# 123456jack/decision-making-and-path-planning

Hardware: AMD Instinct MI355X
Metric: planning ticks/sec (batched scenes), 512x512 grid (higher is better)
Workload: dtype f64; 1 GPU; BASELINE configs[1]: 1024 scenes/GPU, 512x512 grid, 64 static obstacles; scenes_per_gpu=1024, global_scenes=1024, grid=512, obstacles=64, parallelism=scene-sharded x1, RCCL scatter/gather outside the timed region, algorithmic_bytes_per_tick=276644

## Files before the change

### decision-making-and-path-planning_amd/csrc/kernels_s.hpp

```cpp
#pragma once
#include <type_traits>
#include "dev_geom.hpp"

#ifndef DMPP_PRIO_T2
#define DMPP_PRIO_T2 12
#define DMPP_PRIO_T3 36
#endif
namespace dmpp {

__device__ __forceinline__ uint64_t mix64(uint64_t v)
{
    uint64_t z = v + 0x9e3779b97f4a7c15ull;
    z = (z ^ (z >> 30)) * 0xbf58476d1ce4e5b9ull;
    z = (z ^ (z >> 27)) * 0x94d049bb133111ebull;
    return z ^ (z >> 31);
}

__device__ __forceinline__ int index_near(double q)
{
    return (int)fmin(fmax(q, -0x1p30), 0x1p30);
}
__device__ __forceinline__ int index_near_hi(double q)
{
    return (int)fmax(fmin(q, 0x1p30), -0x1p30);
}

__device__ __forceinline__ int cell_of(const PlannerConfig& c, GlobalPoint2D origin, double x, double y)
{
    const int ix = clampi(index_near(floor((x - origin.x) / c.cell)), 0, c.grid_w - 1);
    const int iy = clampi(index_near(floor((y - origin.y) / c.cell)), 0, c.grid_h - 1);
    return iy * c.grid_w + ix;
}

__device__ __forceinline__ int hfun(int x, int y, int gx, int gy)
{
    int dx = abs(x - gx), dy = abs(y - gy);
    return 10 * max(dx, dy) + 4 * min(dx, dy);
}

constexpr int kOpenCap = DMPP_OPEN_CAP;
constexpr uint32_t kEntryForcedA = 1u, kEntryForcedB = 2u, kEntryAheadBlocked = 4u;
template <int K> constexpr int closed_log_of() { return K == 2 ? 10 : 9; }
constexpr int kDiagK = DMPP_DIAG_JUMP;
constexpr int kDiagGroup = 2 * kDiagK;
constexpr int kDiagPerRound = DMPP_WAVE / kDiagGroup;
constexpr int kMaxDiag = 16;
constexpr int kSearchSetupWaves = 4, kSearchBlock = kSearchSetupWaves * DMPP_WAVE;
constexpr int kSearchSetupWavesWide = 16;
constexpr int kOrderShift = 13;
constexpr int kOrderClasses = 1024;

constexpr int kGroupMax = 4;
struct TickGroup {
    int n;
    const SceneIn* in;
    const ObPoint* obs_now; long long obs_stride;
    int32_t* paths; long long path_stride;
    GridOut* gout; long long gout_stride;
};

__device__ __forceinline__ uint32_t wave_min_u32(uint32_t v)
{
#define DMPP_DPP_MIN(ctrl, rowmask)                                                                              \
    { const uint32_t t = (uint32_t)__builtin_amdgcn_update_dpp((int)0xFFFFFFFF, (int)v, ctrl, rowmask, 0xf, false); \
      v = t < v ? t : v; }
    DMPP_DPP_MIN(0x111, 0xf) DMPP_DPP_MIN(0x112, 0xf) DMPP_DPP_MIN(0x114, 0xf) DMPP_DPP_MIN(0x118, 0xf)
    DMPP_DPP_MIN(0x142, 0xa) DMPP_DPP_MIN(0x143, 0xc)
#undef DMPP_DPP_MIN
    return (uint32_t)__builtin_amdgcn_readlane((int)v, 63);
}

__device__ __forceinline__ int popc_m(uint32_t v) { return __popc(v); }
__device__ __forceinline__ int popc_m(uint64_t v) { return __popcll(v); }
__device__ __forceinline__ int lsb_m(uint32_t v) { return __ffs((int)v) - 1; }
__device__ __forceinline__ int lsb_m(uint64_t v) { return __ffsll((long long)v) - 1; }
__device__ __forceinline__ int msb_m(uint32_t v) { return 31 - __clz((int)v); }
__device__ __forceinline__ int msb_m(uint64_t v) { return 63 - __clzll((long long)v); }

constexpr uint32_t kLineOutside = 0xFFFFFFFFu;
template <class M> struct LineM { M mask; uint32_t off; };

#define DMPP_LDS __attribute__((address_space(3)))
template <int K>
struct SparseView {
    using M = std::conditional_t<K == 2, uint64_t, uint32_t>;
    DMPP_LDS uint32_t* data; DMPP_LDS unsigned char* meta; DMPP_LDS uint16_t* off2; int LW, NL;

    __device__ __forceinline__ LineM<M> line(int l) const
    {
        LineM<M> r;
        const bool in = (unsigned)l < (unsigned)NL;
        const int li = in ? l : 0;
        if constexpr (K == 0) { const uint32_t v = ((DMPP_LDS const uint32_t*)meta)[li]; r.mask = v & 0xFFFFu; r.off = v >> 16; }
        else if constexpr (K == 1) { r.mask = ((DMPP_LDS const uint32_t*)meta)[2 * li]; r.off = ((DMPP_LDS const uint32_t*)meta)[2 * li + 1]; }
        else { r.mask = ((DMPP_LDS const uint64_t*)meta)[li]; r.off = off2[li]; }
        if (!in) { r.mask = 0; r.off = kLineOutside; }
        return r;
    }
    __device__ __forceinline__ uint32_t word(const LineM<M>& m, int w) const
    {
        const bool outside = m.off == kLineOutside || (unsigned)w >= (unsigned)LW;
        const M bit = (M)1 << (w & (int)(8 * sizeof(M) - 1));
        const bool present = !outside && (m.mask & bit) != 0;
        const uint32_t idx = present ? m.off + (uint32_t)popc_m((M)(m.mask & (bit - 1))) : 0u;
        const uint32_t v = data[idx];
        return outside ? 0xFFFFFFFFu : (present ? v : 0u);
    }
    __device__ __forceinline__ void clear_line(int l) const
    {
        if constexpr (K == 0) ((DMPP_LDS uint32_t*)meta)[l] = 0;
        else if constexpr (K == 1) { ((DMPP_LDS uint32_t*)meta)[2 * l] = 0; ((DMPP_LDS uint32_t*)meta)[2 * l + 1] = 0; }
        else { ((DMPP_LDS uint64_t*)meta)[l] = 0; off2[l] = (uint16_t)0; }
    }
    __device__ __forceinline__ void or_mask(int l, M bits) const
    {
        if constexpr (K == 0) __hip_atomic_fetch_or(&((DMPP_LDS uint32_t*)meta)[l], (uint32_t)bits, __ATOMIC_RELAXED, __HIP_MEMORY_SCOPE_WORKGROUP);
        else if constexpr (K == 1) __hip_atomic_fetch_or(&((DMPP_LDS uint32_t*)meta)[2 * l], (uint32_t)bits, __ATOMIC_RELAXED, __HIP_MEMORY_SCOPE_WORKGROUP);
        else __hip_atomic_fetch_or(&((DMPP_LDS uint64_t*)meta)[l], (uint64_t)bits, __ATOMIC_RELAXED, __HIP_MEMORY_SCOPE_WORKGROUP);
    }
    __device__ __forceinline__ M mask_of(int l) const
    {
        if constexpr (K == 0) return ((DMPP_LDS const uint32_t*)meta)[l] & 0xFFFFu;
        else if constexpr (K == 1) return ((DMPP_LDS const uint32_t*)meta)[2 * l];
        else return ((DMPP_LDS const uint64_t*)meta)[l];
    }
    __device__ __forceinline__ void set_off(int l, uint32_t off) const
    {
        if constexpr (K == 0) ((DMPP_LDS uint32_t*)meta)[l] |= off << 16;
        else if constexpr (K == 1) ((DMPP_LDS uint32_t*)meta)[2 * l + 1] = off;
        else off2[l] = (uint16_t)off;
    }
};
template <int K> __host__ __device__ constexpr int sparse_meta_bytes_per_line() { return K == 0 ? 4 : (K == 1 ? 8 : 10); }

struct DenseView {
    using M = uint64_t;
    const uint32_t* base; DMPP_LDS const uint64_t* nz; int LW, NL;
    __device__ __forceinline__ LineM<M> line(int l) const
    {
        LineM<M> r; r.mask = 0; r.off = kLineOutside;
        if ((unsigned)l < (unsigned)NL) { r.mask = nz[l]; r.off = (uint32_t)(l * LW); }
        return r;
    }
    __device__ __forceinline__ uint32_t word(const LineM<M>& m, int w) const
    {
        if (m.off == kLineOutside || (unsigned)w >= (unsigned)LW) return 0xFFFFFFFFu;
        if (!((m.mask >> w) & 1ull)) return 0u;
        return base[m.off + w];
    }
};

template <class V>
// ... 573 lines not shown
            ospill[base + r] = make_uint2(L.o_ent[slot], f2 | ((uint32_t)L.o_run[slot] << 16));
            L.o_f2[slot] = 0xFFFFu;
            mn = min(mn, f2);
        }
        base += __popcll(bm);
    }
    sp_n = base;
    sp_min = min(sp_min, wave_min_u32(mn));
    __threadfence();
    wave_order();
    return squeeze_open(L, n_open, lane);
}

template <class LDS>
__device__ __forceinline__ int merge_open(LDS& L, int n_open, int lane, uint2* __restrict__ ospill, int& sp_n, uint32_t& sp_min)
{
    n_open = squeeze_open(L, n_open, lane);
    if (kOpenCap - n_open < 2 * DMPP_WAVE) n_open = spill_open(L, n_open, lane, ospill, sp_n, sp_min);
    __threadfence();
    const uint32_t X = sp_min;
    int cntX = 0;
    for (int q0 = 0; q0 < sp_n; q0 += DMPP_WAVE) {
        const int i = q0 + lane;
        const uint32_t f = i < sp_n ? (ospill[i].y & 0xFFFFu) : 0x10000u;
        cntX += __popcll(wave_ballot(f == X));
    }
    const int room = kOpenCap - n_open - DMPP_WAVE;
    const int take = min(cntX, room), skip = cntX - take;
    {
        uint32_t f2[kOpenCap / DMPP_WAVE], ee[kOpenCap / DMPP_WAVE]; uint16_t rr[kOpenCap / DMPP_WAVE];
#pragma unroll
        for (int k = 0; k < kOpenCap / DMPP_WAVE; k++) {
            const int slot = lane + DMPP_WAVE * k;
            f2[k] = 0xFFFFu; ee[k] = 0; rr[k] = 0;
            if (slot < n_open) { f2[k] = L.o_f2[slot]; ee[k] = L.o_ent[slot]; rr[k] = L.o_run[slot]; }
        }
        wave_order();
#pragma unroll
        for (int k = 0; k < kOpenCap / DMPP_WAVE; k++) {
            const int slot = lane + DMPP_WAVE * k;
            if (slot < n_open) { L.o_f2[slot + take] = (uint16_t)f2[k]; L.o_ent[slot + take] = ee[k]; L.o_run[slot + take] = rr[k]; }
        }
        wave_order();
    }
    int r = 0, w = 0; uint32_t nmin = 0xFFFFu;
    for (int q0 = 0; q0 < sp_n; q0 += DMPP_WAVE) {
        const int i = q0 + lane;
        const bool valid = i < sp_n;
        uint2 e = make_uint2(0u, 0xFFFFu);
        if (valid) e = ospill[i];
        const uint32_t f = e.y & 0xFFFFu;
        const bool isX = valid && f == X;
        const unsigned long long bx = wave_ballot(isX);
        const int myr = r + (int)__builtin_amdgcn_mbcnt_hi((unsigned)(bx >> 32), __builtin_amdgcn_mbcnt_lo((unsigned)bx, 0u));
        const bool tk = isX && myr >= skip;
        if (tk) { const int dst = myr - skip; L.o_f2[dst] = (uint16_t)f; L.o_ent[dst] = e.x; L.o_run[dst] = (uint16_t)(e.y >> 16); }
        const bool kp = valid && !tk;
        const unsigned long long bk = wave_ballot(kp);
        if (kp) {
            ospill[w + (int)__builtin_amdgcn_mbcnt_hi((unsigned)(bk >> 32), __builtin_amdgcn_mbcnt_lo((unsigned)bk, 0u))] = e;
            nmin = min(nmin, f);
        }
        r += __popcll(bx); w += __popcll(bk);
    }
    sp_n = w;
    sp_min = wave_min_u32(nmin);
    __threadfence();
    wave_order();
    return n_open + take;
}

template <bool SPILL, class V, class LDS>
__device__ __forceinline__ SearchOut search_core(const PlannerConfig& c, LDS& L, const V& Vrow, const V& Vcol, int start, int goal, int order_cap,
                                        uint32_t* __restrict__ closed, uint16_t* __restrict__ pin, int32_t* __restrict__ order,
                                        int32_t* __restrict__ path, uint2* __restrict__ ospill, int lane
#ifdef DMPP_DEBUG_SEARCH
                                        , long long* dbg_t, int* dbg_c
#endif
                                        )
{
#ifdef DMPP_DEBUG_SEARCH
#define DBG_MARK(slot) { const long long t__ = clock64(); dbg_t[slot] += t__ - dbg_last; dbg_last = t__; }
    long long dbg_last = clock64();
#else
#define DBG_MARK(slot)
#endif
    constexpr int kClosedLog = LDS::kClosedLog, kClosedTab = LDS::kClosedTab, kClosedMax = LDS::kClosedMax;
    using CW = typename LDS::CW;
    const int W = c.grid_w, H = c.grid_h, N = W * H;
    const int gx = goal % W, gy = goal / W;
    const int cap = SPILL ? c.bucket_cap : min(c.bucket_cap, kOpenCap);
    int sp_n = 0; uint32_t sp_min = 0xFFFFu;
    SearchOut R; R.status = -1; R.n_exp = 0; R.n_push = 1; R.n_rounds = 0; R.path_cost = 0; R.path_len = 0; R.digest = 0;
    int status = -1, n_exp = 0, n_rounds = 0, path_cost = 0;
    int my_pushes = 0;
    uint64_t digest = 0;
    bool hash_complete = true;
    int n_open = 1, live = 1, fmax = -1;
    const int s = lane & 7;
    const int sdx = (s == 0 || s == 1 || s == 7) ? 1 : ((s >= 3 && s <= 5) ? -1 : 0);
    const int sdy = (s >= 1 && s <= 3) ? 1 : ((s >= 5) ? -1 : 0);
    const int node = (lane >> 3) & 3;
    const bool is_dscan = lane < 56, bhv = lane >= 28;
    const int bq = bhv ? lane - 28 : lane;
    const int bj = is_dscan ? bq / 7 : 0, bk = is_dscan ? bq % 7 + 1 : 0;
    const int aj = node, ak = (lane & 7) + 1;
    int guard = 16 * N + 1024;
    int steps = 0;
    while (status < 0) {
        if (__builtin_expect(--guard < 0, 0)) { status = DMPP_G_INTERNAL; break; }
        if (steps == DMPP_PRIO_T2) __builtin_amdgcn_s_setprio(2);
        if (steps == DMPP_PRIO_T3) __builtin_amdgcn_s_setprio(3);
        steps++;
#ifdef DMPP_DEBUG_SEARCH
        dbg_c[0]++;
#endif
        if (__builtin_expect((SPILL ? live + sp_n : live) == 0, 0)) { status = DMPP_G_NO_PATH; break; }
        if (__builtin_expect(n_open - live > 64 && n_open > 2 * live, 0)) n_open = squeeze_open(L, n_open, lane);
        const uint32_t v0 = L.o_f2[lane], v1 = L.o_f2[lane + 64], v2 = L.o_f2[lane + 128], v3 = L.o_f2[lane + 192];
        uint32_t v4 = 0xFFFFu, v5 = 0xFFFFu, v6 = 0xFFFFu, v7 = 0xFFFFu;
        const bool upper = n_open > 256;
        if (__builtin_expect(upper, 0)) { v4 = L.o_f2[lane + 256]; v5 = L.o_f2[lane + 320]; v6 = L.o_f2[lane + 384]; v7 = L.o_f2[lane + 448]; }
        const uint32_t fmin2 = wave_min_u32(min(min(min(v0, v1), min(v2, v3)), min(min(v4, v5), min(v6, v7))));
        if constexpr (SPILL) if (__builtin_expect(sp_n > 0 && fmin2 > sp_min, 0)) { n_open = merge_open(L, n_open, lane, ospill, sp_n, sp_min); live = n_open; continue; }
        if (__builtin_expect(fmin2 == 0xFFFFu, 0)) { status = DMPP_G_INTERNAL; break; }
        const int f = (int)fmin2 << 1;
        int nt = 0; unsigned long long sel = 0;
#define DMPP_TAKE(vreg, base)                                                                        \
        {                                                                                            \
            unsigned long long tm = wave_ballot((vreg) == fmin2);                                    \
            while (tm && nt < DMPP_JPS_BATCH) {                                                      \
                const int b = 63 - __clzll((long long)tm);                                           \
                tm &= ~(1ull << b);                                                                  \
                sel |= (unsigned long long)((base) + b) << (16 * nt);                                \
                nt++;                                                                                \
            }                                                                                        \
        }
        if (__builtin_expect(upper, 0)) { DMPP_TAKE(v7, 448) DMPP_TAKE(v6, 384) DMPP_TAKE(v5, 320) DMPP_TAKE(v4, 256) }
        DMPP_TAKE(v3, 192) DMPP_TAKE(v2, 128) DMPP_TAKE(v1, 64) DMPP_TAKE(v0, 0)
#undef DMPP_TAKE
        static_assert(DMPP_JPS_BATCH == 4 && kOpenCap <= 65536, "four 16-bit slot numbers in one 64-bit scalar");
        if constexpr (SPILL) if (__builtin_expect(sp_n > 0 && fmin2 == sp_min && nt < DMPP_JPS_BATCH, 0)) { n_open = merge_open(L, n_open, lane, ospill, sp_n, sp_min); live = n_open; continue; }
        const int i0 = (int)(sel & 0xFFFFu);
        const int myi = (int)((sel >> (16 * node)) & 0xFFFFu);
        const bool have = lane < 32 && node < nt;
        const uint32_t e = L.o_ent[myi]; const int run_in = L.o_run[myi];
        wave_order();
        if (have && s == 0) L.o_f2[myi] = 0xFFFFu;
        live -= nt;
        n_open -= (i0 == n_open - 1) ? 1 : 0;
        const int x = (int)(e & 0xFFFu), y = (int)((e >> 12) & 0xFFFu), d = (int)((e >> 24) & 15u);
        const uint32_t eflags = e >> 28;
        const int cell = y * W + x;
        DBG_MARK(0)
#ifdef DMPP_DEBUG_SEARCH
        dbg_c[1] += nt;
#endif
        const int gcur = f - hfun(x, y, gx, gy);
        bool jump0, diag0;
        {
            const uint32_t row = d >= 8 ? rules::kCodeStart : (uint32_t)((d < 4 ? rules::kCodeLo : rules::kCodeHi) >> ((d & 3) * 16));
            const uint32_t code = (row >> (2 * s)) & 3u;
            jump0 = code == 1u;
            const int rel = (s - d) & 7;
            const bool forced = ((rel <= 2 ? eflags >> 0 : eflags >> 1) & 1u) != 0;
            const bool ahead_free = (eflags & kEntryAheadBlocked) == 0;
            diag0 = (code == 2u && ahead_free) || (code == 3u && forced);
        }
        DBG_MARK(11)
        bool valid = have && s == 0;
        {
            const int c0_ = __builtin_amdgcn_readlane(cell, 0), c1_ = __builtin_amdgcn_readlane(cell, 8), c2_ = __builtin_amdgcn_readlane(cell, 16);
            const bool dup = ((node >= 1) & (cell == c0_)) | ((node >= 2) & (cell == c1_)) | ((node >= 3) & (cell == c2_));
            valid = valid & !dup;
        }
        uint32_t my_slot = 0;
        if (__builtin_expect(n_exp + DMPP_JPS_BATCH <= kClosedMax, 1)) {
            const uint32_t keyc = (uint32_t)cell + 1u;
            uint32_t hh = ((uint32_t)cell * 2654435761u) >> (32 - kClosedLog);
            uint32_t old = 0u;
            if (valid) old = atomicCAS(&L.c_tab[hh], 0u, keyc);
            if (CW::key(old) == keyc) valid = false;
            bool collide = valid && old != 0u;
            for (int probe = 1; probe < kClosedTab && wave_ballot(collide); probe++) {
                if (collide) {
                    hh = (hh + 1) & (kClosedTab - 1);
                    old = atomicCAS(&L.c_tab[hh], 0u, keyc);
                    if (CW::key(old) == keyc) valid = false;
                    collide = old != 0u && CW::key(old) != keyc;
                }
            }
            my_slot = hh;
        } else {
            if (hash_complete) {
                hash_complete = false;
                digest += hash_digest(L, lane);
                uint4* c4 = reinterpret_cast<uint4*>(closed);
                const uint4 z = { 0u, 0u, 0u, 0u };
                for (int i = lane; i < (N >> 7); i += DMPP_WAVE) c4[i] = z;
                __threadfence();
                wave_sync();
                for (int i = lane; i < kClosedTab; i += DMPP_WAVE) {
                    const uint32_t e2 = L.c_tab[i];
                    if (e2) { const int cc = (int)CW::key(e2) - 1; atomicOr(&closed[cc >> 5], 1u << (cc & 31)); pin[cc] = L.c_info[i]; }
                }
                __threadfence();
                wave_sync();
            }
            if (valid) {
                const uint32_t old = atomicOr(&closed[cell >> 5], 1u << (cell & 31));
                if ((old >> (cell & 31)) & 1u) valid = false;
            }
        }
        const bool inserted = valid;
        auto nodes_of = [](unsigned long long bm) { return (((unsigned)bm & 0x01010101u) * 0x01020408u) >> 24; };
        unsigned vm = nodes_of(wave_ballot(valid));
        {
            const int nvb = __popc(vm & ((1u << node) - 1u));
            const unsigned stop = nodes_of(wave_ballot(valid && (cell == goal || n_exp + nvb + 1 >= c.max_expansions)));
            if (__builtin_expect(stop != 0, 0)) {
                const int last = __ffs((int)stop) - 1;
                if (node > last) valid = false;
                vm = nodes_of(wave_ballot(valid));
            }
        }
        {
            const int seq = n_exp + __popc(vm & ((1u << node) - 1u));
            if (inserted && __builtin_expect(hash_complete, 1)) L.c_info[my_slot] = (uint16_t)(d | (run_in << 4));
            if (valid) {
                if (__builtin_expect(!hash_complete, 0)) { pin[cell] = (uint16_t)(d | (run_in << 4)); digest += mix64(((uint64_t)(uint32_t)seq << 32) | (uint32_t)cell); }
                if (order && seq < order_cap) order[seq] = cell;
            }
            if (inserted && __builtin_expect(hash_complete, 1)) L.set_seq(my_slot, valid ? (uint32_t)seq : CW::kSeqNone);
        }
        if (vm && f > fmax) { fmax = f; n_rounds++; }
        n_exp += __popc(vm);
        if (__builtin_expect(wave_ballot(valid && cell == goal) != 0, 0)) { status = DMPP_G_FOUND; path_cost = f; break; }
        if (__builtin_expect(n_exp >= c.max_expansions, 0)) { status = DMPP_G_LIMIT; break; }
        if (__builtin_expect(vm == 0, 0)) continue;
        DBG_MARK(1)
        const bool nvalid = lane < 32 && ((vm >> node) & 1u);
        const bool want_jump = nvalid && jump0, want_diag = nvalid && diag0;
        int run = 0;
        uint32_t nflags = 0;
        DBG_MARK(2)
        const unsigned smask = (unsigned)wave_ballot(want_jump), dmask = (unsigned)wave_ballot(want_diag);
        const int n_sj = __popc(smask), n_dc = __popc(dmask);
        const int my_sj = __popc(smask & ((1u << (lane & 31)) - 1u)), my_dc = __popc(dmask & ((1u << (lane & 31)) - 1u));
        if (want_jump || want_diag) L.job[want_diag ? my_dc : kMaxDiag + my_sj] = (uint32_t)x | ((uint32_t)y << 12) | ((uint32_t)s << 24);
        wave_order();
        const int n_rounds_j = (n_sj | n_dc) ? max(1, (n_dc + 3) >> 2) : 0;
        DBG_MARK(7)
        for (int rnd = 0; rnd < n_rounds_j; rnd++) {
            const int dca = rnd * 4 + aj;
            const bool a_act = lane < 32 && dca < n_dc;
            const uint32_t Ja = L.job[a_act ? dca : 0];
            const int dcb = rnd * 4 + bj;
            const bool b_act = is_dscan ? dcb < n_dc : (rnd == 0 && lane - 56 < n_sj);
            const uint32_t Jb = L.job[b_act ? (is_dscan ? dcb : kMaxDiag + lane - 56) : 0];
            int jl, jp, jsg; bool hv;
            {
                const int ox = (int)(Jb & 0xFFFu), oy = (int)((Jb >> 12) & 0xFFFu), os = (int)(Jb >> 24);
                if (is_dscan) {
                    const int odx = (os == 1 || os == 7) ? 1 : -1, ody = (os == 1 || os == 3) ? 1 : -1;
                    const int cx = ox + bk * odx, cy = oy + bk * ody;
                    hv = bhv; jl = hv ? cx : cy; jp = hv ? cy : cx; jsg = hv ? ody : odx;
                } else {
                    hv = !(os == 0 || os == 4); jsg = (os == 0 || os == 2) ? 1 : -1; jl = hv ? ox : oy; jp = hv ? oy : ox;
                }
            }
            const V vw = hv ? Vcol : Vrow;
            const int aox = (int)(Ja & 0xFFFu), aoy = (int)((Ja >> 12) & 0xFFFu), aos = (int)(Ja >> 24);
            const int aodx = (aos == 1 || aos == 7) ? 1 : -1, aody = (aos == 1 || aos == 3) ? 1 : -1;
            const int acx = aox + ak * aodx, acy = aoy + ak * aody;
            const auto m0 = vw.line(b_act ? jl : -1), mP = vw.line(b_act ? jl + 1 : -1), mM = vw.line(b_act ? jl - 1 : -1);
            const auto r0 = Vrow.line(a_act ? acy : -1), ra = Vrow.line(a_act ? acy + aody : -1), rb = Vrow.line(a_act ? acy - aody : -1);
            DBG_MARK(8)
            bool cblk = false, cstop = false, cf1 = false, cf2 = false;
            {
                const bool b0 = cell_blocked_m(Vrow, r0, acx), b1 = cell_blocked_m(Vrow, r0, acx - aodx), b2 = cell_blocked_m(Vrow, ra, acx - aodx);
                const bool b3 = cell_blocked_m(Vrow, rb, acx), b4 = cell_blocked_m(Vrow, rb, acx + aodx);
                cf1 = a_act & b1 & !b2;
                cf2 = a_act & b3 & !b4;
                cstop = a_act & (b0 | ((acx == gx) & (acy == gy)) | cf1 | cf2);
                cblk = b0 & a_act;
            }
            DBG_MARK(9)
#ifdef DMPP_DEBUG_SEARCH
            const int r = jump_lane(vw, m0, mP, mM, b_act, jl, jp, jsg, hv ? gx : gy, hv ? gy : gx, &dbg_c[2]);
#else
            const int r = jump_lane(vw, m0, mP, mM, b_act, jl, jp, jsg, hv ? gx : gy, hv ? gy : gx);
#endif
            DBG_MARK(10)
            const unsigned long long am = wave_ballot(cstop), kb = wave_ballot(cblk), sb = wave_ballot(is_dscan && r > 0);
            const unsigned long long f1b = wave_ballot(cf1), f2b = wave_ballot(cf2);
            if (want_diag && (my_dc >> 2) == rnd) {
                const int j = my_dc & 3;
                const unsigned ta = (unsigned)(am >> (8 * j)) & 0xFFu, tk = (unsigned)(kb >> (8 * j)) & 0xFFu;
                const unsigned sc = ((unsigned)(sb >> (7 * j)) | (unsigned)(sb >> (28 + 7 * j))) & 0x7Fu;
                const unsigned any = ta | sc;
                const int k1 = any ? __ffs((int)any) - 1 : kDiagK - 1;
                run = ((tk >> k1) & 1u) ? 0 : k1 + 1;
                const unsigned t1 = ((unsigned)(f1b >> (8 * j)) >> k1) & 1u, t2 = ((unsigned)(f2b >> (8 * j)) >> k1) & 1u;
                const unsigned ahead_blk = (tk >> (k1 + 1)) & 1u;
                const bool ccw_is_1 = s == 1 || s == 5;
                nflags = (ccw_is_1 ? t1 : t2) * kEntryForcedA | (ccw_is_1 ? t2 : t1) * kEntryForcedB | ahead_blk * kEntryAheadBlocked;
            }
            const int from_s = __shfl(r, 56 + (my_sj & 7), 64);
            if (rnd == 0 && want_jump) {
                run = from_s & 0xFFF;
                const unsigned fP = ((unsigned)from_s >> 12) & 1u, fM = ((unsigned)from_s >> 13) & 1u;
                const bool ccw_is_p = s == 0 || s == 6;
                nflags = (ccw_is_p ? fP : fM) * kEntryForcedA | (ccw_is_p ? fM : fP) * kEntryForcedB;
            }
        }
        DBG_MARK(3)
#ifdef DMPP_DEBUG_SEARCH
        dbg_c[3] += n_dc; dbg_c[4] += n_rounds_j;
#endif
        const bool push = run > 0;
        const unsigned pm = (unsigned)wave_ballot(push);
        const int cnt = __popc(pm);
        if (__builtin_expect(cnt != 0, 1)) {
            const int nx = x + run * sdx, ny = y + run * sdy;
            const int fn = gcur + run * ((s & 1) ? 14 : 10) + hfun(nx, ny, gx, gy);
            const unsigned rm = (unsigned)wave_ballot(push && fn >= DMPP_F_LIMIT);
            const int live_all = SPILL ? live + sp_n : live;
            if (__builtin_expect(rm || live_all + cnt > cap, 0)) {
                const int k_range = rm ? __popc(pm & ((1u << (__ffs((int)rm) - 1)) - 1u)) : 0x7FFFFFFF;
                const int k_cap = live_all + cnt > cap ? cap - live_all : 0x7FFFFFFF;
                status = k_range <= k_cap ? DMPP_G_COST_RANGE : DMPP_G_OVERFLOW;
                break;
            }
            if (__builtin_expect(n_open + cnt > kOpenCap, 0)) {
                n_open = squeeze_open(L, n_open, lane);
                if constexpr (SPILL) { if (n_open + cnt > kOpenCap) n_open = spill_open(L, n_open, lane, ospill, sp_n, sp_min); live = n_open; }
            }
            if (push) {
                const int slot = n_open + __popc(pm & ((1u << lane) - 1u));
                L.o_f2[slot] = (uint16_t)(fn >> 1);
                L.o_ent[slot] = (uint32_t)nx | ((uint32_t)ny << 12) | ((uint32_t)s << 24) | (nflags << 28);
                L.o_run[slot] = (uint16_t)run;
            }
            n_open += cnt; live += cnt; my_pushes += push ? 1 : 0;
            wave_order();
        }
        DBG_MARK(4)
    }
    DBG_MARK(5)

    if (hash_complete) digest += hash_digest(L, lane);
#pragma unroll
    for (int sft = 32; sft >= 1; sft >>= 1) {
        uint32_t lo = (uint32_t)digest, hi = (uint32_t)(digest >> 32);
        lo = __shfl_xor((int)lo, sft, 64); hi = __shfl_xor((int)hi, sft, 64);
        digest += ((uint64_t)hi << 32) | lo;
    }
    int path_len = 0;
    bool slow_walk = !hash_complete;
    if (status == DMPP_G_FOUND && hash_complete) {
        int Lc = 1, hops = 0, bad = 0;
        if (lane == 0) {
            int cur = goal;
            while (cur != start) {
                if (hops >= kOpenCap) { bad = 2; break; }
                uint32_t hh = ((uint32_t)cur * 2654435761u) >> (32 - kClosedLog);
                int v = -1;
                for (int probe = 0; probe < kClosedTab; probe++) {
                    const uint32_t e2 = L.c_tab[hh]; const int inf = L.c_info[hh];
                    if (CW::key(e2) == (uint32_t)cur + 1u) { v = inf; break; }
                    if (e2 == 0u) break;
                    hh = (hh + 1) & (kClosedTab - 1);
                }
                const int pd = v & 15, rn = v >> 4;
                if (v < 0 || rn == 0 || pd > 7) { bad = 1; break; }
                const int dx = (int)((0x901Au >> (2 * pd)) & 3u) - 1, dy = (int)((0x01A9u >> (2 * pd)) & 3u) - 1;
                const int step = dy * W + dx;
                L.o_ent[hops] = (uint32_t)cur; L.o_run[hops] = (uint16_t)rn; L.o_f2[hops] = (uint16_t)pd;
                hops++; Lc += rn; cur -= rn * step;
            }
        }
        Lc = __builtin_amdgcn_readfirstlane(Lc);
        hops = __builtin_amdgcn_readfirstlane(hops);
        bad = __builtin_amdgcn_readfirstlane(bad);
        wave_sync();
        if (bad == 1) status = DMPP_G_INTERNAL;
        else if (bad == 2) {
            uint4* c4 = reinterpret_cast<uint4*>(closed);
            (void)c4;
            for (int i = lane; i < kClosedTab; i += DMPP_WAVE) {
                const uint32_t e2 = L.c_tab[i];
                if (e2) pin[(int)CW::key(e2) - 1] = L.c_info[i];
            }
            __threadfence();
            wave_sync();
            slow_walk = true;
        } else {
            int keep = Lc;
            if (Lc > c.max_path) { keep = c.max_path; status = DMPP_G_PATH_TRUNC; }
            path_len = keep;
            int kbase = 0;
            for (int j0 = 0; j0 < hops; j0 += DMPP_WAVE) {
                const int j = j0 + lane;
                const int rn = j < hops ? (int)L.o_run[j] : 0;
                int incl = rn;
#pragma unroll
                for (int sft = 1; sft < DMPP_WAVE; sft <<= 1) { const int t = __shfl_up(incl, sft, 64); if (lane >= sft) incl += t; }
                int ec = 0, step = 0;
                const int idx0 = kbase + incl - rn;
                if (rn) {
                    const int pd = L.o_f2[j];
                    ec = (int)L.o_ent[j];
                    const int dx = (int)((0x901Au >> (2 * pd)) & 3u) - 1, dy = (int)((0x01A9u >> (2 * pd)) & 3u) - 1;
                    step = dy * W + dx;
                }
                constexpr int kLongRun = 12;
                if (rn && rn <= kLongRun) { int idx = idx0; for (int r = 0; r < rn && idx < keep; r++, idx++) path[keep - 1 - idx] = ec - r * step; }
                unsigned long long lm = wave_ballot(rn > kLongRun);
                while (lm) {
                    const int src = __ffsll((long long)lm) - 1;
                    lm &= lm - 1;
                    const int h_ec = __shfl(ec, src, 64), h_step = __shfl(step, src, 64), h_rn = __shfl(rn, src, 64), h_idx = __shfl(idx0, src, 64);
                    for (int r = lane; r < h_rn; r += DMPP_WAVE) if (h_idx + r < keep) path[keep - 1 - (h_idx + r)] = h_ec - r * h_step;
                }
                kbase += __shfl(incl, DMPP_WAVE - 1, 64);
            }
            if (lane == 0 && keep == Lc) path[0] = start;
        }
    }
    if (status == DMPP_G_FOUND && slow_walk) {
        int cur = goal, k = 0;
        bool done = false, broken = false;
        while (!done && !broken) {
            int hops = 0;
            if (lane == 0) {
                int kk = k;
                while (cur != start && hops < kOpenCap) {
                    const int v = pin[cur];
                    const int pd = v & 15, rn = v >> 4;
                    if (rn == 0 || pd > 7 || kk > N) { broken = true; break; }
                    const int dx = (pd == 0 || pd == 1 || pd == 7) ? 1 : ((pd >= 3 && pd <= 5) ? -1 : 0);
                    const int dy = (pd >= 1 && pd <= 3) ? 1 : ((pd >= 5) ? -1 : 0);
                    L.o_ent[hops] = (uint32_t)cur; L.o_run[hops] = (uint16_t)rn; L.o_f2[hops] = (uint16_t)pd;
                    hops++; kk += rn;
                    cur -= rn * (dy * W + dx);
                }
                done = cur == start;
            }
            hops = __builtin_amdgcn_readfirstlane(hops);
            cur = __builtin_amdgcn_readfirstlane(cur);
            done = __builtin_amdgcn_readfirstlane((int)done) != 0;
            broken = __builtin_amdgcn_readfirstlane((int)broken) != 0;
            wave_sync();
            for (int j = 0; j < hops; j++) {
                const int ec = (int)L.o_ent[j], rn = L.o_run[j], pd = L.o_f2[j];
                const int dx = (pd == 0 || pd == 1 || pd == 7) ? 1 : ((pd >= 3 && pd <= 5) ? -1 : 0);
                const int dy = (pd >= 1 && pd <= 3) ? 1 : ((pd >= 5) ? -1 : 0);
                const int step = dy * W + dx;
                for (int r = lane; r < rn; r += DMPP_WAVE)
                    if (k + r < c.max_path) path[k + r] = ec - r * step;
                k += rn;
            }
            wave_sync();
        }
        if (broken) { status = DMPP_G_INTERNAL; }
        else {
            if (lane == 0 && k < c.max_path) path[k] = start;
            const int Lc = k + 1;
            int keep = Lc;
            if (Lc > c.max_path) { keep = c.max_path; status = DMPP_G_PATH_TRUNC; }
            path_len = keep;
            wave_sync();
            for (int i = lane; i < keep / 2; i += DMPP_WAVE) {
                const int a0 = path[i], b0 = path[keep - 1 - i];
                path[i] = b0; path[keep - 1 - i] = a0;
            }
        }
    }
    DBG_MARK(6)
    int n_push = my_pushes;
#pragma unroll
    for (int sft = 32; sft >= 1; sft >>= 1) n_push += __shfl_xor(n_push, sft, 64);
    n_push += 1;
    R.status = status; R.n_exp = n_exp; R.n_push = n_push; R.n_rounds = n_rounds; R.path_cost = path_cost; R.path_len = path_len; R.digest = digest;
    return R;
#undef DBG_MARK
}

template <class LDS>
__device__ __forceinline__ void reset_search_lds(LDS& L, int start, int goal, int W, int lane)
{
    for (int i = lane; i < LDS::kClosedTab; i += DMPP_WAVE) L.c_tab[i] = 0;
    for (int i = lane; i < kOpenCap; i += DMPP_WAVE) L.o_f2[i] = 0xFFFFu;
    wave_order();
    if (lane == 0) {
        const int sx = start % W, sy = start / W;
        L.o_ent[0] = (uint32_t)sx | ((uint32_t)sy << 12) | (8u << 24);
        L.o_f2[0] = (uint16_t)(hfun(sx, sy, goal % W, goal / W) >> 1);
        L.o_run[0] = 0;
    }
    wave_order();
}

__device__ __forceinline__ void publish_search(GridOut& go, const SearchOut& R, int start, int goal)
{
    go.order_digest = R.digest; go.status = R.status; go.n_expanded = R.n_exp; go.n_pushed = R.n_push; go.n_rounds = R.n_rounds;
    go.path_len = R.path_len; go.path_cost = R.path_cost; go.start_cell = start; go.goal_cell = goal;
}

#ifdef DMPP_DEBUG_SEARCH
__device__ __forceinline__ void publish_debug(int32_t* path, int max_path, const long long* t, const int* cn, long long t_setup, long long t_total)
{
    int32_t* dbg = path + max_path - 16;
    dbg[0] = cn[0]; dbg[1] = cn[1]; dbg[2] = cn[2]; dbg[3] = cn[3]; dbg[4] = cn[4];
    dbg[5] = (int)(t[0] >> 4); dbg[6] = (int)(t[1] >> 4); dbg[7] = (int)(t[2] >> 4); dbg[8] = (int)(t[3] >> 4); dbg[9] = (int)(t[4] >> 4);
    dbg[10] = (int)(t[6] >> 4); dbg[11] = (int)((t[0] + t[1] + t[2] + t[3] + t[4] + t[5] + t[6]) >> 4); dbg[12] = (int)(t_setup >> 4); dbg[13] = (int)(t_total >> 4);
    dbg[14] = (int)__builtin_amdgcn_s_getreg((31 << 11) | 4);
    dbg[15] = (int)__builtin_amdgcn_s_getreg((31 << 11) | 20);
    for (int i = 7; i < 16; i++) path[max_path - 64 + i] = (int)(t[i] >> 4);
}
#endif

template <int K, int SW, bool SPILL>
__device__ __forceinline__ void search_scene(const PlannerConfig& c, int scene, int w_base, int order_cap, int budget, const SceneIn* __restrict__ in,
         const ObPoint* __restrict__ obs_now, uint32_t* __restrict__ gclosed, uint16_t* __restrict__ pinfo, int32_t* __restrict__ orders,
         int32_t* __restrict__ paths, GridOut* __restrict__ gout, uint32_t* __restrict__ gbitmaps, int32_t* __restrict__ cost_out,
         int32_t* __restrict__ overflow, int32_t* __restrict__ need_max, uint2* __restrict__ ospill_all, int spill_cap,
         int32_t* __restrict__ retry_list, int32_t* __restrict__ retry_cnt,
         SearchLds<closed_log_of<K>()>& L, unsigned char* smem_raw)
{
    using LdsT = SearchLds<closed_log_of<K>()>;
    constexpr unsigned kViewsAt = 0;
    const long long t_begin = clock64();
    const int tid = threadIdx.x, lane = tid & (DMPP_WAVE - 1), wv = tid >> 6;
    const int W = c.grid_w, H = c.grid_h, N = W * H, WW = W >> 5, HW = H >> 5;
    const SceneIn& si = in[scene];
    SparseView<K> vr, vc;
    {
        DMPP_LDS unsigned char* p = (DMPP_LDS unsigned char*)smem_raw + kViewsAt;
        unsigned used = 0;
        if constexpr (K == 2) {
            vr.meta = p; vc.meta = p + (unsigned)H * 8u;
            vr.off2 = (DMPP_LDS uint16_t*)(p + (unsigned)(H + W) * 8u); vc.off2 = vr.off2 + H;
            used = (unsigned)(H + W) * 10u;
        } else {
            constexpr unsigned mb = (unsigned)sparse_meta_bytes_per_line<K>();
            vr.meta = p; vc.meta = p + (unsigned)H * mb;
            vr.off2 = nullptr; vc.off2 = nullptr;
            used = (unsigned)(H + W) * mb;
        }
        used = (used + 15u) & ~15u;
        vr.data = (DMPP_LDS uint32_t*)(p + used); vc.data = vr.data + budget;
        vr.LW = WW; vr.NL = H; vc.LW = HW; vc.NL = W;
    }
    static_assert(sizeof(RasterStage) <= offsetof(LdsT, job), "the staged footprints must fit the open list and the closed set");
    DMPP_LDS RasterStage* stage = (DMPP_LDS RasterStage*)(DMPP_LDS unsigned char*)(unsigned char*)&L;
    int* s_wave2 = (int*)L.job;
    static_assert(sizeof(L.job) >= kSearchSetupWavesWide * sizeof(int), "second row of wave sums");
    const ObPoint* obs = obs_now + si.obs_off;
#ifdef DMPP_DEBUG_SEARCH
    long long tmark[8] = { 0, 0, 0, 0, 0, 0, 0, 0 };
    const int need = budget > 0 ? build_sparse_views<K, SW>(c, si, obs, si.obs_n, vr, vc, budget, stage, L.s_wave, s_wave2, tmark) : 1;
#else
    const int need = budget > 0 ? build_sparse_views<K, SW>(c, si, obs, si.obs_n, vr, vc, budget, stage, L.s_wave, s_wave2) : 1;
#endif
    const bool dense = need > budget;
    if (tid == 0) { if (budget > 0) atomicMax(need_max, need); overflow[scene] = dense ? 1 : 0; }
    uint32_t* bm = gbitmaps + (size_t)scene * 2 * (N >> 5);
    DMPP_LDS uint64_t* nz_row = (DMPP_LDS uint64_t*)((DMPP_LDS unsigned char*)smem_raw + kViewsAt);
    DMPP_LDS uint64_t* nz_col = nz_row + H;
    if (dense) { __syncthreads(); build_dense_views<SW>(c, si, obs, si.obs_n, bm, nz_row, nz_col, stage, L.s_wave); }
    for (int i = tid; i < LdsT::kClosedTab; i += (SW * DMPP_WAVE)) L.c_tab[i] = 0;
    for (int i = tid; i < kOpenCap; i += (SW * DMPP_WAVE)) L.o_f2[i] = 0xFFFFu;
    const DenseView dr{ bm, nz_row, WW, H }, dc{ bm + (N >> 5), nz_col, HW, W };
    const int start = cell_of(c, si.grid_origin, si.loc.globalpoint.x, si.loc.globalpoint.y);
    const int goal = cell_of(c, si.grid_origin, si.goal.x, si.goal.y);
    const bool goal_blocked = dense ? cell_blocked(dr, goal % W, goal / W) : cell_blocked(vr, goal % W, goal / W);
    __syncthreads();
    if (!goal_blocked && tid == 0) {
        const int sx = start % W, sy = start / W;
        if (dense) {
            bm[start >> 5] &= ~(1u << (start & 31));
            bm[(N >> 5) + sx * HW + (sy >> 5)] &= ~(1u << (sy & 31));
            __threadfence();
        } else {
            sparse_clear_cell(vr, sy, sx);
            sparse_clear_cell(vc, sx, sy);
        }
        L.o_ent[0] = (uint32_t)sx | ((uint32_t)sy << 12) | (8u << 24);
        L.o_f2[0] = (uint16_t)(hfun(sx, sy, goal % W, goal / W) >> 1);
        L.o_run[0] = 0;
    }
    __syncthreads();
    int32_t* path = paths + (size_t)scene * c.max_path;
    if (wv != 0) return;
    __builtin_amdgcn_s_setprio(1);
    const long long t_setup = clock64() - t_begin;
    SearchOut R; R.status = DMPP_G_GOAL_BLOCKED; R.n_exp = 0; R.n_push = 0; R.n_rounds = 0; R.path_cost = 0; R.path_len = 0; R.digest = 0;
    uint32_t* closed = gclosed + (size_t)scene * (N >> 5);
    uint16_t* pin = pinfo + (size_t)scene * N;
    int32_t* order = orders ? orders + (size_t)scene * order_cap : nullptr;
    uint2* ospill = ospill_all ? ospill_all + (size_t)scene * spill_cap : nullptr;
// ... 128 lines not shown
```

Measured before the change: 6.382 million ticks/s.

## Parallelize path reconstruction via wave-wide parent-slot table and DPP reductions

Replaces the serial lane-0 hash-probing walk from goal to start with a wave-parallel pass. That pass compacts the occupied closed-hash slots and resolves each slot's parent slot into LDS reused from the open-list arrays, and it also computes the digest in the same sweep. The lane-0 walk then only follows precomputed parent indices, and run lengths and cell coordinates are re-read from the hash table. Shuffle-based reductions and scans are replaced with DPP-based wave scans and sums. The cost is that every search now resolves parents for all occupied slots, not just the ones on the path, and the open-list LDS is aliased for the new tables.

New measurement: 6.487 million ticks/s, median of 6. 1.02x the previous value.

```diff
diff --git a/decision-making-and-path-planning_amd/csrc/kernels_s.hpp b/decision-making-and-path-planning_amd/csrc/kernels_s.hpp
--- a/decision-making-and-path-planning_amd/csrc/kernels_s.hpp
+++ b/decision-making-and-path-planning_amd/csrc/kernels_s.hpp
@@ -68,6 +68,28 @@
     DMPP_DPP_MIN(0x142, 0xa) DMPP_DPP_MIN(0x143, 0xc)
 #undef DMPP_DPP_MIN
     return (uint32_t)__builtin_amdgcn_readlane((int)v, 63);
+}
+
+__device__ __forceinline__ int wave_scan_i32(int v)
+{
+#define DMPP_DPP_ADD(ctrl, rowmask) v += __builtin_amdgcn_update_dpp(0, v, ctrl, rowmask, 0xf, false);
+    DMPP_DPP_ADD(0x111, 0xf) DMPP_DPP_ADD(0x112, 0xf) DMPP_DPP_ADD(0x114, 0xf) DMPP_DPP_ADD(0x118, 0xf)
+    DMPP_DPP_ADD(0x142, 0xa) DMPP_DPP_ADD(0x143, 0xc)
+#undef DMPP_DPP_ADD
+    return v;
+}
+__device__ __forceinline__ int wave_sum_i32(int v) { return __builtin_amdgcn_readlane(wave_scan_i32(v), 63); }
+__device__ __forceinline__ uint64_t wave_sum_u64(uint64_t v)
+{
+#define DMPP_DPP_ADD64(ctrl, rowmask)                                                                             \
+    { const uint32_t lo = (uint32_t)__builtin_amdgcn_update_dpp(0, (int)(uint32_t)v, ctrl, rowmask, 0xf, false);      \
+      const uint32_t hi = (uint32_t)__builtin_amdgcn_update_dpp(0, (int)(uint32_t)(v >> 32), ctrl, rowmask, 0xf, false); \
+      v += ((uint64_t)hi << 32) | lo; }
+    DMPP_DPP_ADD64(0x111, 0xf) DMPP_DPP_ADD64(0x112, 0xf) DMPP_DPP_ADD64(0x114, 0xf) DMPP_DPP_ADD64(0x118, 0xf)
+    DMPP_DPP_ADD64(0x142, 0xa) DMPP_DPP_ADD64(0x143, 0xc)
+#undef DMPP_DPP_ADD64
+    const uint32_t lo = (uint32_t)__builtin_amdgcn_readlane((int)(uint32_t)v, 63), hi = (uint32_t)__builtin_amdgcn_readlane((int)(uint32_t)(v >> 32), 63);
+    return ((uint64_t)hi << 32) | lo;
 }
 
 __device__ __forceinline__ int popc_m(uint32_t v) { return __popc(v); }
@@ -807,6 +829,7 @@
 #ifdef DMPP_DEBUG_SEARCH
 #define DBG_MARK(slot) { const long long t__ = clock64(); dbg_t[slot] += t__ - dbg_last; dbg_last = t__; }
     long long dbg_last = clock64();
+    int hops_dbg = 0;
 #else
 #define DBG_MARK(slot)
 #endif
@@ -821,6 +844,7 @@
     int my_pushes = 0;
     uint64_t digest = 0;
     bool hash_complete = true;
+    uint32_t goal_slot = 0;
     int n_open = 1, live = 1, fmax = -1;
     const int s = lane & 7;
     const int sdx = (s == 0 || s == 1 || s == 7) ? 1 : ((s >= 3 && s <= 5) ? -1 : 0);
@@ -960,7 +984,14 @@
         }
         if (vm && f > fmax) { fmax = f; n_rounds++; }
         n_exp += __popc(vm);
-        if (__builtin_expect(wave_ballot(valid && cell == goal) != 0, 0)) { status = DMPP_G_FOUND; path_cost = f; break; }
+        {
+            const unsigned long long at_goal = wave_ballot(valid && cell == goal);
+            if (__builtin_expect(at_goal != 0, 0)) {
+                status = DMPP_G_FOUND; path_cost = f;
+                goal_slot = (uint32_t)__builtin_amdgcn_readlane((int)my_slot, __ffsll((long long)at_goal) - 1);
+                break;
+            }
+        }
         if (__builtin_expect(n_exp >= c.max_expansions, 0)) { status = DMPP_G_LIMIT; break; }
         if (__builtin_expect(vm == 0, 0)) continue;
         DBG_MARK(1)
@@ -1074,41 +1105,84 @@
     }
     DBG_MARK(5)
 
-    if (hash_complete) digest += hash_digest(L, lane);
-#pragma unroll
-    for (int sft = 32; sft >= 1; sft >>= 1) {
-        uint32_t lo = (uint32_t)digest, hi = (uint32_t)(digest >> 32);
-        lo = __shfl_xor((int)lo, sft, 64); hi = __shfl_xor((int)hi, sft, 64);
-        digest += ((uint64_t)hi << 32) | lo;
-    }
     int path_len = 0;
     bool slow_walk = !hash_complete;
-    if (status == DMPP_G_FOUND && hash_complete) {
+    constexpr uint32_t kParStart = 0xFFFDu, kParInvalid = 0xFFFEu, kParMissing = 0xFFFFu;
+    typedef uint16_t __attribute__((may_alias)) u16_alias;
+    u16_alias* const par = reinterpret_cast<u16_alias*>(L.o_ent);
+    u16_alias* const occ = reinterpret_cast<u16_alias*>(L.o_f2);
+    static_assert(kClosedTab < (int)kParStart && sizeof(L.o_ent) >= kClosedTab * sizeof(uint16_t) && sizeof(L.o_f2) >= kOpenCap * sizeof(uint16_t) &&
+                  offsetof(LDS, o_run) == offsetof(LDS, o_f2) + sizeof(L.o_f2) && sizeof(L.o_f2) + sizeof(L.o_run) >= kClosedTab * sizeof(uint16_t),
+                  "parent slots over o_ent, occupied slots over o_f2 | o_run, the hop list over o_f2");
+    const bool chain = status == DMPP_G_FOUND && hash_complete;
+    const uint32_t start_slot = ((uint32_t)start * 2654435761u) >> (32 - kClosedLog);
+    if (hash_complete) {
+        int n_occ = 0;
+        {
+            constexpr int NS = kClosedTab / DMPP_WAVE;
+            uint32_t E[NS];
+#pragma unroll
+            for (int k = 0; k < NS; k++) E[k] = L.c_tab[lane + k * DMPP_WAVE];
+            wave_order();
+#pragma unroll
+            for (int k = 0; k < NS; k++) {
+                const bool o = E[k] != 0u;
+                const unsigned long long bm = wave_ballot(o);
+                if (o) occ[n_occ + (int)__builtin_amdgcn_mbcnt_hi((unsigned)(bm >> 32), __builtin_amdgcn_mbcnt_lo((unsigned)bm, 0u))] = (uint16_t)(lane + k * DMPP_WAVE);
+                n_occ += __popcll(bm);
+            }
+            wave_order();
+        }
+        for (int r0 = 0; r0 < n_occ; r0 += DMPP_WAVE) {
+            const bool act = r0 + lane < n_occ;
+            const uint32_t sl = act ? (uint32_t)occ[r0 + lane] : 0u;
+            const uint32_t e = L.c_tab[sl], inf = L.c_info[sl]; const uint32_t sq = L.seq_of(sl, e);
+            if (act && sq != CW::kSeqNone) digest += mix64(((uint64_t)sq << 32) | (uint64_t)(CW::key(e) - 1u));
+            if (chain) {
+                const int pd = (int)(inf & 15u), rn = (int)(inf >> 4);
+                const int dx = (int)((0x901Au >> (2 * (pd & 7))) & 3u) - 1, dy = (int)((0x01A9u >> (2 * (pd & 7))) & 3u) - 1;
+                const bool want = act && pd <= 7 && rn > 0;
+                const uint32_t keyc = CW::key(e) - (uint32_t)(rn * (dy * W + dx));
+                uint32_t hh = ((keyc - 1u) * 2654435761u) >> (32 - kClosedLog);
+                uint32_t e2 = L.c_tab[hh];
+                bool miss = want && CW::key(e2) != keyc && e2 == 0u, coll = want && CW::key(e2) != keyc && e2 != 0u;
+                for (int probe = 1; probe < kClosedTab && wave_ballot(coll); probe++) {
+                    if (coll) {
+                        hh = (hh + 1u) & (uint32_t)(kClosedTab - 1);
+                        e2 = L.c_tab[hh];
+                        if (CW::key(e2) == keyc) coll = false;
+                        else if (e2 == 0u) { coll = false; miss = true; }
+                    }
+                }
+                miss |= coll;
+                if (act) par[sl] = (uint16_t)(!want ? kParInvalid : (miss ? kParMissing : (hh == start_slot ? kParStart : hh)));
+            }
+        }
+        wave_order();
+    }
+    DBG_MARK(12)
+    digest = wave_sum_u64(digest);
+    DBG_MARK(15)
+    if (chain) {
         int Lc = 1, hops = 0, bad = 0;
-        if (lane == 0) {
-            int cur = goal;
-            while (cur != start) {
+        if (lane == 0 && goal_slot != start_slot) {
+            uint32_t cur = goal_slot;
+            for (;;) {
+                L.o_f2[hops] = (uint16_t)cur;
+                hops++;
+                const uint32_t up = (uint32_t)__builtin_amdgcn_readfirstlane((int)par[cur]);
+                if (up >= kParStart) { bad = up == kParStart ? 0 : 1; break; }
                 if (hops >= kOpenCap) { bad = 2; break; }
-                uint32_t hh = ((uint32_t)cur * 2654435761u) >> (32 - kClosedLog);
-                int v = -1;
-                for (int probe = 0; probe < kClosedTab; probe++) {
-                    const uint32_t e2 = L.c_tab[hh]; const int inf = L.c_info[hh];
-                    if (CW::key(e2) == (uint32_t)cur + 1u) { v = inf; break; }
-                    if (e2 == 0u) break;
-                    hh = (hh + 1) & (kClosedTab - 1);
-                }
-                const int pd = v & 15, rn = v >> 4;
-                if (v < 0 || rn == 0 || pd > 7) { bad = 1; break; }
-                const int dx = (int)((0x901Au >> (2 * pd)) & 3u) - 1, dy = (int)((0x01A9u >> (2 * pd)) & 3u) - 1;
-                const int step = dy * W + dx;
-                L.o_ent[hops] = (uint32_t)cur; L.o_run[hops] = (uint16_t)rn; L.o_f2[hops] = (uint16_t)pd;
-                hops++; Lc += rn; cur -= rn * step;
-            }
-        }
-        Lc = __builtin_amdgcn_readfirstlane(Lc);
+                cur = up;
+            }
+        }
         hops = __builtin_amdgcn_readfirstlane(hops);
         bad = __builtin_amdgcn_readfirstlane(bad);
         wave_sync();
+        DBG_MARK(13)
+#ifdef DMPP_DEBUG_SEARCH
+        hops_dbg = hops;
+#endif
         if (bad == 1) status = DMPP_G_INTERNAL;
         else if (bad == 2) {
             uint4* c4 = reinterpret_cast<uint4*>(closed);
@@ -1121,36 +1195,39 @@
             wave_sync();
             slow_walk = true;
         } else {
+            uint32_t e_first = 0, i_first = 0;
+            if (lane < hops) { const int sl = L.o_f2[lane]; e_first = L.c_tab[sl]; i_first = L.c_info[sl]; }
+            int runs = (int)(i_first >> 4);
+            for (int j = DMPP_WAVE + lane; j < hops; j += DMPP_WAVE) runs += (int)(L.c_info[L.o_f2[j]] >> 4);
+            Lc = 1 + wave_sum_i32(runs);
             int keep = Lc;
             if (Lc > c.max_path) { keep = c.max_path; status = DMPP_G_PATH_TRUNC; }
             path_len = keep;
             int kbase = 0;
             for (int j0 = 0; j0 < hops; j0 += DMPP_WAVE) {
                 const int j = j0 + lane;
-                const int rn = j < hops ? (int)L.o_run[j] : 0;
-                int incl = rn;
-#pragma unroll
-                for (int sft = 1; sft < DMPP_WAVE; sft <<= 1) { const int t = __shfl_up(incl, sft, 64); if (lane >= sft) incl += t; }
-                int ec = 0, step = 0;
+                uint32_t e2 = e_first, inf = i_first;
+                if (j0) { e2 = 0; inf = 0; if (j < hops) { const int sl = L.o_f2[j]; e2 = L.c_tab[sl]; inf = L.c_info[sl]; } }
+                const int rn = (int)(inf >> 4), pd = (int)(inf & 15u);
+                const int incl = wave_scan_i32(rn);
                 const int idx0 = kbase + incl - rn;
-                if (rn) {
-                    const int pd = L.o_f2[j];
-                    ec = (int)L.o_ent[j];
-                    const int dx = (int)((0x901Au >> (2 * pd)) & 3u) - 1, dy = (int)((0x01A9u >> (2 * pd)) & 3u) - 1;
-                    step = dy * W + dx;
-                }
+                const int ec = (int)CW::key(e2) - 1;
+                const int dx = (int)((0x901Au >> (2 * pd)) & 3u) - 1, dy = (int)((0x01A9u >> (2 * pd)) & 3u) - 1;
+                const int step = dy * W + dx;
                 constexpr int kLongRun = 12;
                 if (rn && rn <= kLongRun) { int idx = idx0; for (int r = 0; r < rn && idx < keep; r++, idx++) path[keep - 1 - idx] = ec - r * step; }
                 unsigned long long lm = wave_ballot(rn > kLongRun);
                 while (lm) {
                     const int src = __ffsll((long long)lm) - 1;
                     lm &= lm - 1;
-                    const int h_ec = __shfl(ec, src, 64), h_step = __shfl(step, src, 64), h_rn = __shfl(rn, src, 64), h_idx = __shfl(idx0, src, 64);
+                    const int h_ec = __builtin_amdgcn_readlane(ec, src), h_step = __builtin_amdgcn_readlane(step, src);
+                    const int h_rn = __builtin_amdgcn_readlane(rn, src), h_idx = __builtin_amdgcn_readlane(idx0, src);
                     for (int r = lane; r < h_rn; r += DMPP_WAVE) if (h_idx + r < keep) path[keep - 1 - (h_idx + r)] = h_ec - r * h_step;
                 }
-                kbase += __shfl(incl, DMPP_WAVE - 1, 64);
+                kbase += __builtin_amdgcn_readlane(incl, DMPP_WAVE - 1);
             }
             if (lane == 0 && keep == Lc) path[0] = start;
+            DBG_MARK(14)
         }
     }
     if (status == DMPP_G_FOUND && slow_walk) {
@@ -1203,10 +1280,12 @@
         }
     }
     DBG_MARK(6)
-    int n_push = my_pushes;
-#pragma unroll
-    for (int sft = 32; sft >= 1; sft >>= 1) n_push += __shfl_xor(n_push, sft, 64);
-    n_push += 1;
+    const int n_push = wave_sum_i32(my_pushes) + 1;
+    DBG_MARK(15)
+#ifdef DMPP_DEBUG_SEARCH
+    dbg_t[6] += dbg_t[12] + dbg_t[13] + dbg_t[14] + dbg_t[15];
+    dbg_c[5] = hops_dbg;
+#endif
     R.status = status; R.n_exp = n_exp; R.n_push = n_push; R.n_rounds = n_rounds; R.path_cost = path_cost; R.path_len = path_len; R.digest = digest;
     return R;
 #undef DBG_MARK
@@ -1243,6 +1322,7 @@
     dbg[14] = (int)__builtin_amdgcn_s_getreg((31 << 11) | 4);
     dbg[15] = (int)__builtin_amdgcn_s_getreg((31 << 11) | 20);
     for (int i = 7; i < 16; i++) path[max_path - 64 + i] = (int)(t[i] >> 4);
+    path[max_path - 64 + 6] = cn[5];
 }
 #endif
 
```
